# aravindr93/mjrl

Measured on AMD Instinct MI355X. Metric: NPG updates/sec (1M-timestep batch, 64x64 MLP), higher is better.
Workload: dtype f32; 1 GPU; BASELINE configs[1]: HalfCheetah-v2 shapes (obs=17, act=6), 64x64 tanh MLP, NPG 10 CG iters, 1M timesteps/batch (1000 traj x 1000), device-resident update; global_batch=1000000, parallelism=dp1 (trajectory shards, one rank sum per CG iteration: none at one rank), cg_iters=10

## Files before the change

mjrl_amd/csrc/fused_policy.h:

```cpp
#pragma once
#include <hip/hip_runtime.h>
#include <stdint.h>

#include <type_traits>
#include <vector>

namespace mjx {

typedef float f32x16 __attribute__((ext_vector_type(16)));
typedef float f32x4 __attribute__((ext_vector_type(4)));
typedef float f32x2 __attribute__((ext_vector_type(2)));

enum { MODE_VPG = 0, MODE_FVP = 1, MODE_EVAL = 2 };

struct FusedArgs {
  const float* obs;
  const float* act;
  const float* adv;
  int64_t N;
  float inv_N;
  const float* thetaA;
  const float* thetaB;
  const float* trA;
  const float* trB;
  int old_is_new;
  float* partials;
  double* spartials;
  float* dbg;
  long long* clk;
  int reverse;
  float* hcache;
  float* ocache;
  const float* snap;
  int snap_trusted;
  float* snap_out;
  int n, m;
  int raw_dr;
};

#ifdef MJX_PHASE_CLOCK
#define MJX_STAMP(k) do { __builtin_amdgcn_sched_barrier(0); if (A.dbg && blockIdx.x == 0 && wave == 0 && lane == 0 && tile == tstride) ((long long*)A.dbg)[k] = (long long)__builtin_readcyclecounter(); __builtin_amdgcn_sched_barrier(0); } while (0)
#else
#define MJX_STAMP(k) do {} while (0)
#endif
#ifdef MJX_PHASE_CLOCK
#define MJX_GSTAMP(k) do { if (A.dbg && blockIdx.x == 0 && threadIdx.x == 0) { ((long long*)A.dbg)[k] = (long long)__builtin_readcyclecounter(); ((long long*)A.dbg)[(k) + 8] = (long long)__builtin_amdgcn_s_memrealtime(); } } while (0)
#else
#define MJX_GSTAMP(k) do {} while (0)
#endif
#define MJX_MFMA(a, b, c) __builtin_amdgcn_mfma_f32_32x32x2f32((a), (b), (c), 0, 0, 0)
#define MJX_MFMA_ACC(acc, a, b) asm volatile("v_mfma_f32_32x32x2_f32 %0, %1, %2, %0" : "+a"(acc) : "v"(a), "v"(b))
#define MJX_MFMA4_ACC(acc, a, b) asm volatile("v_mfma_f32_4x4x1_16b_f32 %0, %1, %2, %0" : "+a"(acc) : "v"(a), "v"(b))
typedef __attribute__((address_space(3))) float lds_float;
__device__ __forceinline__ uint32_t lds_pin(const float* p) {
  uint32_t a = (uint32_t)(uintptr_t)(const lds_float*)p;
  asm volatile("" : "+v"(a));
  return a;
}
#define LDS_AT(addr) ((lds_float*)(uintptr_t)(addr))
#define LDS_ST(p, v) (*(p) = (v))
#define LDS_LD(p) (*(p))
#define LDS_LD2(p) (*(const f32x2*)(p))

__device__ __forceinline__ void wave_sync() {
  __builtin_amdgcn_fence(__ATOMIC_RELEASE, "wavefront");
  __builtin_amdgcn_wave_barrier();
  __builtin_amdgcn_fence(__ATOMIC_ACQUIRE, "wavefront");
}

__device__ __forceinline__ float fast_tanh(float x) {
  const float d = 1.0f + __builtin_amdgcn_exp2f(x * 2.885390081777927f);
  return fmaf(__builtin_amdgcn_rcpf(d), -2.0f, 1.0f);
}

__device__ __forceinline__ void fast_tanh16(f32x16& o, const f32x16& x) {
#pragma unroll
  for (int r = 0; r < 16; r += 2) {
    const f32x2 s = f32x2{x[r], x[r + 1]} * (f32x2)(2.885390081777927f);
    const f32x2 d = f32x2{__builtin_amdgcn_exp2f(s.x), __builtin_amdgcn_exp2f(s.y)} + (f32x2)(1.0f);
    const f32x2 rr = {__builtin_amdgcn_rcpf(d.x), __builtin_amdgcn_rcpf(d.y)};
    const f32x2 y = __builtin_elementwise_fma(rr, (f32x2)(-2.0f), (f32x2)(1.0f));
    o[r] = y.x; o[r + 1] = y.y;
  }
}

__device__ __forceinline__ float fast_div(float a, float b) {
  float r = __builtin_amdgcn_rcpf(b);
  r = r * fmaf(-b, r, 2.0f);
  return a * r;
}

__device__ __forceinline__ float half_select(uint32_t mask, float a, float b) {
  return __uint_as_float((__float_as_uint(a) & mask) | (__float_as_uint(b) & ~mask));
}

__device__ __forceinline__ float half_sum(float p) {
  auto s = __builtin_amdgcn_permlane32_swap(__float_as_uint(p), __float_as_uint(p), false, false);
  return __uint_as_float(s[0]) + __uint_as_float(s[1]);
}

__device__ __forceinline__ float row16_sum(float v) {
  auto dpp = [](float x, auto ctrl) {
    return __int_as_float(__builtin_amdgcn_update_dpp(0, __float_as_int(x), decltype(ctrl)::value, 0xF, 0xF, true));
  };
  v += dpp(v, std::integral_constant<int, 0xB1>{});
  v += dpp(v, std::integral_constant<int, 0x4E>{});
  v += dpp(v, std::integral_constant<int, 0x141>{});
  v += dpp(v, std::integral_constant<int, 0x140>{});
  return v;
}

__device__ __forceinline__ f32x16 pk_1mh2(const f32x16& h) {
  f32x16 o;
#pragma unroll
  for (int r = 0; r < 16; r += 2) {
    const f32x2 hh = {h[r], h[r + 1]};
    const f32x2 ff = __builtin_elementwise_fma(-hh, hh, (f32x2)(1.0f));
    o[r] = ff.x; o[r + 1] = ff.y;
  }
  return o;
}
__device__ __forceinline__ void pk_mul(f32x16& t, const f32x16& f) {
#pragma unroll
  for (int r = 0; r < 16; r += 2) {
    f32x2 tt = {t[r], t[r + 1]};
    tt *= f32x2{f[r], f[r + 1]};
    t[r] = tt.x; t[r + 1] = tt.y;
  }
}
__device__ __forceinline__ void pk_mul_1mh2(f32x16& t, const f32x16& h) {
#pragma unroll
  for (int r = 0; r < 16; r += 2) {
    const f32x2 hh = {h[r], h[r + 1]};
    f32x2 tt = {t[r], t[r + 1]};
    tt *= __builtin_elementwise_fma(-hh, hh, (f32x2)(1.0f));
    t[r] = tt.x; t[r + 1] = tt.y;
  }
}
__device__ __forceinline__ f32x2 pk_1mh2_pair_far(f32x2 hh) {
  f32x2 ff;
  asm("v_pk_fma_f32 %0, %1, %1, 1.0 op_sel_hi:[1,1,0] neg_lo:[1,0,0] neg_hi:[1,0,0]" : "=v"(ff) : "v"(hh));
  return ff;
}
__device__ __forceinline__ f32x16 pk_1mh2_far(const f32x16& h) {
  f32x16 o;
#pragma unroll
  for (int r = 0; r < 16; r += 2) {
    const f32x2 ff = pk_1mh2_pair_far(f32x2{h[r], h[r + 1]});
    o[r] = ff.x; o[r + 1] = ff.y;
  }
  return o;
}
__device__ __forceinline__ f32x2 mul_1mh2_pair(float a0, float a1, float h0, float h1) {
  const f32x2 ff = pk_1mh2_pair_far(f32x2{h0, h1});
  f32x2 tt = {a0, a1};
  tt *= ff;
  return tt;
}
__device__ __forceinline__ void pk_mul_1mh2_far(f32x16& t, const f32x16& h) {
#pragma unroll
  for (int r = 0; r < 16; r += 2) {
    f32x2 tt = {t[r], t[r + 1]};
    const f32x2 ff = pk_1mh2_pair_far(f32x2{h[r], h[r + 1]});
    asm("v_pk_mul_f32 %0, %0, %1" : "+v"(tt) : "v"(ff));
    t[r] = tt.x; t[r + 1] = tt.y;
  }
}

typedef __bf16 bf16x8 __attribute__((ext_vector_type(8)));
typedef uint32_t u32x4 __attribute__((ext_vector_type(4)));
#define MJX_MFMA_BF16(a, b, c) __builtin_amdgcn_mfma_f32_32x32x16_bf16(__builtin_bit_cast(bf16x8, (a)), __builtin_bit_cast(bf16x8, (b)), (c), 0, 0, 0)
struct Pc3 { u32x4 p[3]; };
__device__ __forceinline__ Pc3 split3(const float (&x)[8]) {
  Pc3 o;
#pragma unroll
  for (int k = 0; k < 4; ++k) {
    const uint32_t ua = __float_as_uint(x[2 * k]), ub = __float_as_uint(x[2 * k + 1]);
    const float ra = x[2 * k] - __uint_as_float(ua & 0xffff0000u), rb = x[2 * k + 1] - __uint_as_float(ub & 0xffff0000u);
    const uint32_t va = __float_as_uint(ra), vb = __float_as_uint(rb);
    const float la = ra - __uint_as_float(va & 0xffff0000u), lb = rb - __uint_as_float(vb & 0xffff0000u);
    o.p[0][k] = __builtin_amdgcn_perm(ub, ua, 0x07060302u);
    o.p[1][k] = __builtin_amdgcn_perm(vb, va, 0x07060302u);
    o.p[2][k] = __builtin_amdgcn_perm(__float_as_uint(lb), __float_as_uint(la), 0x07060302u);
  }
  return o;
}
__device__ __forceinline__ Pc3 split3_of(const f32x16& v, int s) {
  float x[8];
#pragma unroll
  for (int i = 0; i < 8; ++i) x[i] = v[8 * s + i];
  return split3(x);
}
__device__ __forceinline__ f32x16 mfma_bf3(const Pc3& a, const Pc3& b, f32x16 c) {
  c = MJX_MFMA_BF16(a.p[2], b.p[0], c);
  c = MJX_MFMA_BF16(a.p[0], b.p[2], c);
  c = MJX_MFMA_BF16(a.p[1], b.p[1], c);
  c = MJX_MFMA_BF16(a.p[1], b.p[0], c);
  c = MJX_MFMA_BF16(a.p[0], b.p[1], c);
  c = MJX_MFMA_BF16(a.p[0], b.p[0], c);
  return c;
}

template <int N, int I = 0, class F>
__device__ __forceinline__ void static_for(F&& f) {
  if constexpr (I < N) { f(std::integral_constant<int, I>{}); static_for<N, I + 1>(f); }
}

__device__ __forceinline__ constexpr int unit_of(int r, int hi) { return (r & 3) + 8 * (r >> 2) + 4 * hi; }

template <int H1, int H2, int NT1, int MP>
struct FusedLayout {
  static constexpr int MT1 = H1 / 32, MT2 = H2 / 32;
  static constexpr int S2 = H1 + 4;
  static constexpr int ST = 36;
  static constexpr int S3 = H2 + 4;
  static constexpr int HM = (H1 > H2 ? H1 : H2);
  int NP;
  int S1;
  int oW1, oW2, oW3, oB2, oB3, SLOT;
  int oXS, oXT, oD3, oBA, oBB, WAVE;
  int oTR, oCST, oWAVES, TOTAL;
  static constexpr int NCST = 13;
  static constexpr int F2_IMG = 3 * H1 * H2 / 2;
  __host__ __device__ explicit FusedLayout(int n, bool eval_only = false, bool bf3 = false) {
    NP = (n + 1 + 3) & ~3;
    S1 = NP + 2;
    oW1 = 0;
    oW2 = oW1 + H1 * S1;
    oW3 = oW2 + ((bf3 && H2 * S2 < F2_IMG) ? F2_IMG : H2 * S2);
    oB2 = oW3 + MP * S3;
    oB3 = oB2 + H2;
    SLOT = ((oB3 + MP + 3) / 4) * 4;
    oXS = 0;
    oXT = bf3 ? 0 : ((oXS + 32 * n + 4 * 64 + 3) / 4) * 4;
    oD3 = oXT + NP * ST;
    oBA = oD3 + MP * ST;
    oBB = oBA + HM * ST;
    WAVE = eval_only ? ((oXT + 3) / 4) * 4 : ((oBB + HM * ST + 3) / 4) * 4;
    oTR = 2 * SLOT;
    oCST = oTR + 4 * NP;
    oWAVES = oCST + NCST * MP;
    TOTAL = oWAVES + 4 * WAVE;
  }
  __host__ __device__ size_t bytes() const { return (size_t)TOTAL * 4; }
  __host__ __device__ bool fits(int n) const { return n + 1 <= 32 * NT1; }
};

struct FlatOff {
  int W1, b1, W2, b2, W3, b3, S, d;
  __host__ __device__ FlatOff(int n, int m, int h1, int h2) {
    W1 = 0; b1 = W1 + h1 * n; W2 = b1 + h1; b2 = W2 + h2 * h1; W3 = b2 + h2; b3 = W3 + m * h2; S = b3 + m; d = S + m;
  }
};

template <int H1, int H2, int NT1, int MP, int NPC>
struct RawSlab {
  static constexpr int MT1 = H1 / 32, MT2 = H2 / 32, RA = MP / 2;
  static constexpr int QPI3 = 16 / (MP / 4), UPI3 = 4 * QPI3, NT3 = H2 / UPI3;
  static constexpr int NFQ = NPC ? NPC / 4 : 1;
  static constexpr int oW2 = 0, nW2 = MT2 * MT1 * 16 * 64;
  static constexpr int oW1 = oW2 + nW2, nW1 = NPC ? MT1 * NFQ * 4 * 32 : MT1 * NT1 * 16 * 64;
  static constexpr int oW3 = oW1 + nW1, nW3 = NT3 * 4 * 64;
  static constexpr int oB2 = oW3 + nW3, nB2 = MT2 * 32;
  static constexpr int oB3 = oB2 + nB2;
  static constexpr int oS = oB3 + 2 * RA;
  static constexpr int DR = ((oS + 2 * RA) + 3) & ~3;
  static int unit(int r, int hi) { return (r & 3) + 8 * (r >> 2) + 4 * hi; }
  static bool fill_perm(int* perm, int n, int m) {
    const FlatOff fo(n, m, H1, H2);
    for (int i = 0; i < DR; ++i) perm[i] = -1;
    auto w1 = [&](int u, int f) { return f < n ? fo.W1 + u * n + f : f == n ? fo.b1 + u : -1; };
    for (int mt = 0; mt < MT2; ++mt) for (int nt = 0; nt < MT1; ++nt) for (int r = 0; r < 16; ++r) for (int l = 0; l < 64; ++l)
      perm[oW2 + ((mt * MT1 + nt) * 16 + r) * 64 + l] = fo.W2 + (32 * mt + unit(r, l >> 5)) * H1 + 32 * nt + (l & 31);
    if (NPC) {
      for (int mt = 0; mt < MT1; ++mt) for (int fq = 0; fq < NFQ; ++fq) for (int r = 0; r < 4; ++r) for (int l = 0; l < 32; ++l)
        perm[oW1 + ((mt * NFQ + fq) * 4 + r) * 32 + l] = w1(32 * mt + 4 * ((l >> 2) & 7) + r, 4 * fq + (l & 3));
    } else {
      for (int mt = 0; mt < MT1; ++mt) for (int nt = 0; nt < NT1; ++nt) for (int r = 0; r < 16; ++r) for (int l = 0; l < 64; ++l)
        perm[oW1 + ((mt * NT1 + nt) * 16 + r) * 64 + l] = w1(32 * mt + unit(r, l >> 5), 32 * nt + (l & 31));
    }
    for (int nt = 0; nt < NT3; ++nt) for (int r = 0; r < 4; ++r) for (int l = 0; l < 64; ++l) {
      const int blk = l >> 2, a = 4 * (blk / QPI3) + r, u = 4 * (blk % QPI3) + (l & 3) + UPI3 * nt;
      perm[oW3 + (nt * 4 + r) * 64 + l] = a < m ? fo.W3 + a * H2 + u : -1;
    }
    for (int nt = 0; nt < MT2; ++nt) for (int jj = 0; jj < 32; ++jj) perm[oB2 + nt * 32 + jj] = fo.b2 + 32 * nt + jj;
    for (int r = 0; r < RA; ++r) for (int hi = 0; hi < 2; ++hi) {
      const int a = unit(r, hi);
      perm[oB3 + 2 * r + hi] = a < m ? fo.b3 + a : -1;
      perm[oS + 2 * r + hi] = a < m ? fo.S + a : -1;
    }
    std::vector<int> hits(fo.d, 0);
    for (int i = 0; i < DR; ++i) if (perm[i] >= 0) { if (perm[i] >= fo.d) return false; ++hits[perm[i]]; }
    for (int i = 0; i < fo.d; ++i) if (hits[i] != 1) return false;
    return true;
  }
};

template <int H1, int H2, int NT1, int MP, int MODE, bool DBG = false, int NPC = 0, bool CACHED = false, bool BF3 = false>
__global__ __launch_bounds__(256, (MODE == MODE_EVAL && !DBG && MP <= 8) ? 2 : 1) void k_fused(FusedArgs A) {
  using LT = FusedLayout<H1, H2, NT1, MP>;
  constexpr int MT1 = LT::MT1, MT2 = LT::MT2, S2 = LT::S2, S3 = LT::S3, ST = LT::ST;
  constexpr int RA = MP / 2;
  extern __shared__ __attribute__((aligned(16))) float lds[];
  const int tid = threadIdx.x, lane = tid & 63, j = lane & 31, hi = lane >> 5;
  const int wave = __builtin_amdgcn_readfirstlane(tid >> 6);
  const uint32_t himask = hi ? 0xffffffffu : 0u;
  const int n = A.n, m = A.m;
  constexpr bool EV2 = (MODE == MODE_EVAL) && !DBG && MP <= 8;
  constexpr bool XBF3 = (MODE == MODE_FVP) && CACHED && BF3;
  static_assert(!BF3 || (CACHED && MODE == MODE_FVP && H1 == 64 && H2 == 64), "bf16x3: the cached 64 x 64 Fisher-vector product only");
  const LT L(NPC ? NPC - 1 : n, EV2, XBF3);
  const int NP = NPC ? NPC : L.NP;
  const int S1 = NP + 2;
  const FlatOff fo(n, m, H1, H2);

  float* slotA = lds;
  float* slotB = lds + L.SLOT;
  float* trs = lds + L.oTR;
  float* ws = lds + L.oWAVES + wave * L.WAVE;
  float* xs = ws + L.oXS;
  float* xT = ws + L.oXT;
  float* d3T = ws + L.oD3;
  float* bufA = ws + L.oBA;
  float* bufB = ws + L.oBB;

  MJX_GSTAMP(16);
  if (A.clk && blockIdx.x == 0 && threadIdx.x == 0) { A.clk[0] = (long long)__builtin_readcyclecounter(); A.clk[1] = (long long)__builtin_amdgcn_s_memrealtime(); }
  constexpr bool XCACHED = (MODE == MODE_FVP) && CACHED;
  constexpr int C1 = NPC ? NPC / 4 : 8 * NT1;
  constexpr int C2 = (H2 * H1 / 4 + 255) / 256;
  constexpr int C3 = (MP * H2 + 255) / 256;
  const int u1 = tid >> 2, p1 = tid & 3;
  float w1r[2][C1], w3r[2][C3], b2r[2], b3r[2], trr[4], csr[7];
  f32x4 w2r[2][C2];
#pragma unroll
  for (int s = 0; s < 2; ++s) {
    const float* th = s ? A.thetaB : A.thetaA;
    if (!(XCACHED && s == 0)) {
#pragma unroll
      for (int c = 0; c < C1; ++c) {
        const int f = p1 + 4 * c;
        const bool ok = (u1 < H1) && (f <= n);
        w1r[s][c] = th[ok ? ((f < n) ? fo.W1 + u1 * n + f : fo.b1 + u1) : 0];
      }
    }
#pragma unroll
    for (int c = 0; c < C2; ++c) { const int i4 = c * 256 + tid; w2r[s][c] = *(const f32x4*)&th[fo.W2 + 4 * (i4 < H2 * H1 / 4 ? i4 : 0)]; }
#pragma unroll
    for (int c = 0; c < C3; ++c) { const int idx = c * 256 + tid; w3r[s][c] = th[fo.W3 + (idx < m * H2 ? idx : 0)]; }
    b2r[s] = th[fo.b2 + (tid < H2 ? tid : 0)];
    b3r[s] = th[fo.b3 + (tid < m ? tid : 0)];
  }
  {
    const int i = tid < n ? tid : 0;
    trr[0] = A.trA[i]; trr[1] = A.trA[n + i]; trr[2] = A.trB[i]; trr[3] = A.trB[n + i];
    const int a = tid < m ? tid : 0;
    csr[0] = A.thetaA[fo.S + a]; csr[1] = A.thetaB[fo.S + a];
    csr[2] = A.trA[2 * n + m + a]; csr[3] = A.trA[2 * n + a];
    csr[4] = A.trB[2 * n + m + a]; csr[5] = A.trB[2 * n + a];
    csr[6] = A.thetaB[fo.b3 + a];
  }
  int mism = 0, mismx = 0;
  if (MODE == MODE_EVAL && A.ocache && !A.snap_trusted) {
    for (int idx = tid; idx < fo.d; idx += 256) mism |= (A.thetaB[idx] != A.snap[idx]);
    for (int idx = tid; idx < 2 * (n + m); idx += 256) mism |= (A.trB[idx] != A.snap[fo.d + idx]);
    if (A.hcache) for (int idx = tid; idx < 2 * n; idx += 256) mismx |= (A.trA[idx] != A.snap[fo.d + idx]);
  }
  if (MODE == MODE_VPG && A.snap_out) {
    const int nsnap = fo.d + 2 * (n + m);
    for (int idx = blockIdx.x * 256 + tid; idx < nsnap; idx += gridDim.x * 256)
      A.snap_out[idx] = idx < fo.d ? A.thetaB[idx] : A.trB[idx - fo.d];
  }
  {
    f32x4* z4 = (f32x4*)lds;
    for (int i = tid; i < L.oWAVES / 4; i += 256) z4[i] = (f32x4)(0.f);
    f32x4* w4 = (f32x4*)ws;
    for (int i = lane; i < (EV2 ? L.WAVE : L.oBA) / 4; i += 64) w4[i] = (f32x4)(0.f);
  }
  __syncthreads();
#pragma unroll
  for (int s = 0; s < 2; ++s) {
    float* slot = s ? slotB : slotA;
    if (!(XCACHED && s == 0)) {
#pragma unroll
      for (int c = 0; c < C1; ++c) {
        const int f = p1 + 4 * c;
        if ((u1 < H1) && (f <= n)) slot[L.oW1 + u1 * S1 + f] = w1r[s][c];
      }
    }
#pragma unroll
    for (int c = 0; c < C2; ++c) {
      const int i4 = c * 256 + tid;
      if (i4 < H2 * H1 / 4) *(f32x4*)&slot[L.oW2 + ((4 * i4) / H1) * S2 + (4 * i4) % H1] = w2r[s][c];
    }
#pragma unroll
    for (int c = 0; c < C3; ++c) {
      const int idx = c * 256 + tid;
      if (idx < m * H2) slot[L.oW3 + (idx / H2) * S3 + idx % H2] = w3r[s][c];
    }
    if (tid < H2) slot[L.oB2 + tid] = b2r[s];
    if (tid < m) slot[L.oB3 + tid] = b3r[s];
  }
  if (tid < n) { trs[tid] = trr[0]; trs[NP + tid] = 1.0f / (trr[1] + 1e-8f); trs[2 * NP + tid] = trr[2]; trs[3 * NP + tid] = 1.0f / (trr[3] + 1e-8f); }
  if (!EV2 && lane < 32) xT[n * ST + lane] = 1.0f;

  float* cst = lds + L.oCST;
  enum { C_OSC = 0, C_OSH = 1, C_SG = 2, C_LS = 3, C_OSCB = 4, C_OSHB = 5, C_SGB = 6, C_LSB = 7, C_DK = 8, C_ISG = 11, C_ISGB = 12,
         C_RD = 8, C_SO2 = 9, C_SN2 = 10, C_KD = 2 };
  if (tid < MP) {
    const int a = tid;
    const bool ok = a < m;
    const float lsa = ok ? csr[0] : 0.f;
    const float lsb = (ok && MODE != MODE_FVP) ? csr[1] : lsa;
    const float sga = ok ? expf(lsa) : 1.0f;
    const float dk = 2.0f / (2.0f * sga * sga + 1e-8f);
    cst[C_OSC * MP + a] = ok ? csr[2] : 0.f;
    cst[C_OSH * MP + a] = ok ? csr[3] : 0.f;
    cst[C_SG * MP + a] = sga;
    cst[C_LS * MP + a] = lsa;
    cst[C_OSCB * MP + a] = ok ? csr[4] : 0.f;
    cst[C_OSHB * MP + a] = ok ? csr[5] : 0.f;
    cst[C_SGB * MP + a] = ok ? expf(lsb) : 1.0f;
    cst[C_LSB * MP + a] = lsb;
    cst[C_DK * MP + a] = dk;
    cst[C_ISG * MP + a] = ok ? 1.0f / sga : 0.f;
    cst[C_ISGB * MP + a] = ok ? 1.0f / cst[C_SGB * MP + a] : 0.f;
    if (MODE == MODE_EVAL) {
      const float sgb = cst[C_SGB * MP + a];
      const float Dr = 2.0f * sga * sga + 1e-8f;
      float r = __builtin_amdgcn_rcpf(Dr);
      r = r * fmaf(-Dr, r, 2.0f);
      cst[C_RD * MP + a] = r;
      cst[C_SO2 * MP + a] = sgb * sgb;
      cst[C_SN2 * MP + a] = sga * sga;
      cst[C_KD * MP + a] = lsa - lsb;
    }
    if (MODE == MODE_FVP) {
      const float osc = ok ? csr[2] : 0.f;
      cst[9 * MP + 2 * a] = ok ? csr[6] : 0.f;
      cst[9 * MP + 2 * a + 1] = osc * (dk * (osc * A.inv_N));
    }
  }
  if (MODE == MODE_EVAL && mism) lds[L.oWAVES] = 1.0f;
  if (MODE == MODE_EVAL && mismx) lds[L.oWAVES + 1] = 1.0f;
  __syncthreads();
  bool use_oc = false, use_xi = false;
  if (MODE == MODE_EVAL && A.ocache) {
    use_oc = (lds[L.oWAVES] == 0.0f);
    use_xi = use_oc && NPC != 0 && A.hcache != nullptr && (lds[L.oWAVES + 1] == 0.0f);
    __syncthreads();
  }
  Pc3 w3p[XBF3 ? MT2 : 1][XBF3 ? MT1 : 1][2];
  if constexpr (XBF3) {
#pragma unroll
    for (int mt = 0; mt < MT2; ++mt)
#pragma unroll
      for (int kb = 0; kb < MT1; ++kb)
#pragma unroll
        for (int s = 0; s < 2; ++s) {
          const float* row = &slotA[L.oW2 + (32 * mt + j) * S2 + 32 * kb + 16 * s + 4 * hi];
          const f32x4 a = *(const f32x4*)row, b = *(const f32x4*)(row + 8);
          const float x[8] = {a.x, a.y, a.z, a.w, b.x, b.y, b.z, b.w};
          w3p[mt][kb][s] = split3(x);
// ... 481 lines not shown
      MJX_STAMP(6);
      f32x16 dl2s[MT2];
#pragma unroll
      for (int mt = 0; mt < MT2; ++mt) dl2s[mt] = (f32x16)(0.f);
#pragma unroll
      for (int sidx = 0; sidx < RA; ++sidx)
#pragma unroll
        for (int mt = 0; mt < MT2; ++mt) dl2s[mt] = MJX_MFMA(w6[sidx][mt], d3r[sidx], dl2s[mt]);
      float wc8[4][MT1];
      {
        const int blk = lane >> 2, g3 = blk / QPI3, uq3 = blk % QPI3;
        const float* arow = &d3T[(4 * g3 + (lane & 3)) * ST];
        const float* brow = &bufA[(4 * uq3 + (lane & 3)) * ST];
#pragma unroll
        for (int sp = 0; sp < 4; ++sp) {
          const f32x4 ave = *(const f32x4*)(arow + 8 * sp), avo = *(const f32x4*)(arow + 8 * sp + 4);
          f32x4 bve[NT3], bvo[NT3];
#pragma unroll
          for (int nt = 0; nt < NT3; ++nt) { bve[nt] = *(const f32x4*)(brow + UPI3 * nt * ST + 8 * sp); bvo[nt] = *(const f32x4*)(brow + UPI3 * nt * ST + 8 * sp + 4); }
#pragma unroll
          for (int t = 0; t < 4; ++t)
#pragma unroll
            for (int nt = 0; nt < NT3; ++nt) {
              gW3[nt] = __builtin_amdgcn_mfma_f32_4x4x1f32(ave[t], bve[nt][t], gW3[nt], 0, 0, 0);
              gW3b[nt] = __builtin_amdgcn_mfma_f32_4x4x1f32(avo[t], bvo[nt][t], gW3b[nt], 0, 0, 0);
            }
        }
        if constexpr (!XBF3) {
#pragma unroll
          for (int t = 0; t < 4; ++t)
#pragma unroll
            for (int nt = 0; nt < MT1; ++nt) wc8[t][nt] = LDS_AT(pinW[0])[t * S2 + 32 * nt];
        }
      }
      __builtin_amdgcn_sched_barrier(0);
      MJX_STAMP(7);
#pragma unroll
      for (int mt = 0; mt < MT2; ++mt) pk_mul(dl2s[mt], f2s[mt]);
      f32x16 dl1u[MT1];
      float dl2u[MT2][16];
#pragma unroll
      for (int nt = 0; nt < MT1; ++nt) dl1u[nt] = (f32x16)(0.f);
      if constexpr (XBF3) {
        __builtin_amdgcn_sched_barrier(0);
        load_h(ptile((tile + tstride < ntiles) ? tile + tstride : tile));
        const u32x4* img = (const u32x4*)(slotA + L.oW2) + lane;
        constexpr int NG8 = 2 * MT2;
        Pc3 ac = split3_of(dl2s[0], 0), an = ac, bc[MT1], bn[MT1];
#pragma unroll
        for (int nt = 0; nt < MT1; ++nt)
#pragma unroll
          for (int p = 0; p < 3; ++p) bc[nt].p[p] = img[(p * 8 + nt * 4) * 64];
        __builtin_amdgcn_sched_barrier(0);
#pragma unroll
        for (int g = 0; g < NG8; ++g) {
          if (g + 1 < NG8) {
            const int kb1 = (g + 1) >> 1, s1 = (g + 1) & 1;
#pragma unroll
            for (int nt = 0; nt < MT1; ++nt)
#pragma unroll
              for (int p = 0; p < 3; ++p) bn[nt].p[p] = img[(p * 8 + (nt * 2 + kb1) * 2 + s1) * 64];
            an = split3_of(dl2s[kb1], s1);
          }
#pragma unroll
          for (int nt = 0; nt < MT1; ++nt) dl1u[nt] = mfma_bf3(ac, bc[nt], dl1u[nt]);
          if (g < MT2) {
#pragma unroll
            for (int r = 0; r < 16; ++r) LDS_AT(pinA[4 * g + (r >> 2)])[(r & 3) * ST] = dl2s[g][r];
          } else {
            const int nt = g - MT2;
#pragma unroll
            for (int qq = 0; qq < 4; ++qq) {
              const f32x4 v = *(const f32x4*)&bufA[(32 * nt + j) * ST + 8 * qq + 4 * hi];
              dl2u[nt][4 * qq] = v.x; dl2u[nt][4 * qq + 1] = v.y; dl2u[nt][4 * qq + 2] = v.z; dl2u[nt][4 * qq + 3] = v.w;
            }
          }
          ac = an;
#pragma unroll
          for (int nt = 0; nt < MT1; ++nt) bc[nt] = bn[nt];
        }
#pragma unroll
        for (int g = 0; g < NG8; ++g)
#pragma unroll
          for (int i = 0; i < 6 * MT1; ++i) {
            __builtin_amdgcn_sched_group_barrier(0x008, 1, 0);
            if (g + 1 < NG8) {
              __builtin_amdgcn_sched_group_barrier(0x002, 4, 0);
              if (i < 3 * MT1) __builtin_amdgcn_sched_group_barrier(0x100, 1, 0);
            }
            if (g < MT2) { if (i < 4) __builtin_amdgcn_sched_group_barrier(0x200, 2, 0); else __builtin_amdgcn_sched_group_barrier(0x200, 1, 0); }
            else if (i < 4) __builtin_amdgcn_sched_group_barrier(0x100, 1, 0);
          }
        __builtin_amdgcn_sched_barrier(0);
      } else {
        constexpr int NG = MT2 * 4;
        constexpr int NGH = NG / 2;
        float wc[4][MT1], wn[4][MT1];
        __builtin_amdgcn_sched_barrier(0);
        load_h(ptile((tile + tstride < ntiles) ? tile + tstride : tile));
#pragma unroll
        for (int t = 0; t < 4; ++t)
#pragma unroll
          for (int nt = 0; nt < MT1; ++nt) wc[t][nt] = wc8[t][nt];
#pragma unroll
        for (int g = 0; g < NG; ++g) {
          const int kb = g >> 2, q = g & 3;
          if (g + 1 < NG) {
            const int kb1 = (g + 1) >> 2, q1 = (g + 1) & 3;
#pragma unroll
            for (int t = 0; t < 4; ++t)
#pragma unroll
              for (int nt = 0; nt < MT1; ++nt) wn[t][nt] = LDS_AT(pinW[4 * kb1 + q1])[t * S2 + 32 * nt];
          }
#pragma unroll
          for (int t = 0; t < 4; ++t)
#pragma unroll
            for (int nt = 0; nt < MT1; ++nt) dl1u[nt] = MJX_MFMA(dl2s[kb][4 * q + t], wc[t][nt], dl1u[nt]);
          if (g < NGH) {
            constexpr int RS = 16 * MT2 / NGH;
#pragma unroll
            for (int e = 0; e < RS; ++e) {
              const int idx = g * RS + e, mt = idx >> 4, r = idx & 15;
              LDS_AT(pinA[4 * mt + (r >> 2)])[(r & 3) * ST] = dl2s[mt][r];
            }
          } else {
            constexpr int RQ = (4 * MT2 + NGH - 1) / NGH;
#pragma unroll
            for (int e = 0; e < RQ; ++e) {
              const int idx = (g - NGH) * RQ + e;
              if (idx < 4 * MT2) {
                const int nt = idx >> 2, qq = idx & 3;
                const f32x4 v = *(const f32x4*)&bufA[(32 * nt + j) * ST + 8 * qq + 4 * hi];
                dl2u[nt][4 * qq] = v.x; dl2u[nt][4 * qq + 1] = v.y; dl2u[nt][4 * qq + 2] = v.z; dl2u[nt][4 * qq + 3] = v.w;
              }
            }
          }
#pragma unroll
          for (int t = 0; t < 4; ++t)
#pragma unroll
            for (int nt = 0; nt < MT1; ++nt) wc[t][nt] = wn[t][nt];
        }
#pragma unroll
        for (int g = 0; g < NG; ++g) {
          if (g + 1 < NG) __builtin_amdgcn_sched_group_barrier(0x100, 2 * MT1, 0);
#pragma unroll
          for (int i = 0; i < 4 * MT1; ++i) {
            __builtin_amdgcn_sched_group_barrier(0x008, 1, 0);
            if (g < NGH) __builtin_amdgcn_sched_group_barrier(0x200, 1, 0);
            else if (i < (4 * MT2 + NGH - 1) / NGH) __builtin_amdgcn_sched_group_barrier(0x100, 1, 0);
          }
        }
      }
      f32x4 bcs[4][MT1];
#pragma unroll
      for (int nt = 0; nt < MT1; ++nt) bcs[0][nt] = *(const f32x4*)&bufB[(32 * nt + j) * ST + 4 * hi];
      __builtin_amdgcn_sched_barrier(0);
      MJX_STAMP(8);
      {
#pragma unroll
        for (int q = 1; q < 4; ++q)
#pragma unroll
          for (int nt = 0; nt < MT1; ++nt) bcs[q][nt] = *(const f32x4*)&bufB[(32 * nt + j) * ST + 8 * q + 4 * hi];
#pragma unroll
        for (int q = 0; q < 4; ++q) {
#pragma unroll
          for (int t = 0; t < 4; ++t)
#pragma unroll
            for (int mt = 0; mt < MT2; ++mt)
#pragma unroll
              for (int nt = 0; nt < MT1; ++nt) MJX_MFMA_ACC(gW2[mt][nt], dl2u[mt][4 * q + t], bcs[q][nt][t]);
        }
        __builtin_amdgcn_sched_barrier(0);
      }
      MJX_STAMP(9);
#pragma unroll
      for (int nt = 0; nt < MT1; ++nt)
#pragma unroll
        for (int q = 0; q < 4; ++q)
#pragma unroll
          for (int t = 0; t < 4; t += 2) {
            const f32x2 hh = {bcs[q][nt][t], bcs[q][nt][t + 1]};
            f32x2 dd = {dl1u[nt][4 * q + t], dl1u[nt][4 * q + t + 1]};
            dd *= __builtin_elementwise_fma(-hh, hh, (f32x2)(1.0f));
            dl1u[nt][4 * q + t] = dd.x; dl1u[nt][4 * q + t + 1] = dd.y;
          }
#pragma unroll
      for (int nt = 0; nt < MT2; ++nt) {
        f32x2 s2 = {dl2u[nt][0], dl2u[nt][1]};
#pragma unroll
        for (int r = 2; r < 16; r += 2) s2 += f32x2{dl2u[nt][r], dl2u[nt][r + 1]};
        sb2[nt] += s2.x + s2.y;
      }
      __builtin_amdgcn_sched_barrier(0);
      if constexpr (NPC != 0) {
        const float* xrow = &xT[(lane & 3) * ST + 4 * hi];
#pragma unroll
        for (int q = 0; q < 4; ++q) {
          f32x4 bx[NFQ];
#pragma unroll
          for (int fq = 0; fq < NFQ; ++fq) bx[fq] = *(const f32x4*)(xrow + 4 * fq * ST + 8 * q);
#pragma unroll
          for (int t = 0; t < 4; ++t)
#pragma unroll
            for (int fq = 0; fq < NFQ; ++fq)
#pragma unroll
              for (int mt = 0; mt < MT1; ++mt)
                MJX_MFMA4_ACC(gW1q[mt][fq], dl1u[mt][4 * q + t], bx[fq][t]);
        }
      } else {
        f32x4 bc[NT1], bn[NT1];
#pragma unroll
        for (int nt = 0; nt < NT1; ++nt) { int f = 32 * nt + j; bc[nt] = *(const f32x4*)&xT[(f < NP ? f : 0) * ST + 4 * hi]; }
#pragma unroll
        for (int q = 0; q < 4; ++q) {
          if (q + 1 < 4) {
#pragma unroll
            for (int nt = 0; nt < NT1; ++nt) { int f = 32 * nt + j; bn[nt] = *(const f32x4*)&xT[(f < NP ? f : 0) * ST + 8 * (q + 1) + 4 * hi]; }
          }
#pragma unroll
          for (int nt = 0; nt < NT1; ++nt) {
            f32x4 b4 = (32 * nt + j < NP) ? bc[nt] : (f32x4)(0.f);
#pragma unroll
            for (int t = 0; t < 4; ++t)
#pragma unroll
              for (int mt = 0; mt < MT1; ++mt) gW1[mt][nt] = MJX_MFMA(dl1u[mt][4 * q + t], b4[t], gW1[mt][nt]);
          }
#pragma unroll
          for (int nt = 0; nt < NT1; ++nt) bc[nt] = bn[nt];
        }
      }
      MJX_STAMP(13);
      __builtin_amdgcn_sched_barrier(0);
    } else {
    float actr[MP], advr = 0.f;
    if (MODE != MODE_FVP) {
      if (s0 + 32 + MP <= A.N) {
        gcptr ab = ubase(A.act + s0 * m);
        gcptr db = ubase(A.adv + s0);
#pragma unroll
        for (int a = 0; a < MP; ++a) actr[a] = *(const float __attribute__((address_space(1)))*)(ab + aoff + 4 * a);
        advr = *(const float __attribute__((address_space(1)))*)(db + (uint32_t)(j * 4));
      } else {
#pragma unroll
        for (int a = 0; a < MP; ++a) actr[a] = A.act[(valid && a < m) ? (s0 + j) * m + a : 0];
        advr = A.adv[valid ? s0 + j : 0];
      }
    }
    if constexpr (DIRX) {
      const int64_t tn = tile + tstride;
      if (tn < ntiles) {
        if ((tn + 1) * 32 > A.N) set_xoff(xo, (tn * 32 + j < A.N) ? (uint32_t)j : 0u);
        load_xw(xw, xo, tn);
      }
      if (A.hcache) {
        gwptr xb = (gwptr)ubase(A.hcache + tile * HC_TILE + HC_H);
#pragma unroll
        for (int q = 0; q < NQX; ++q) *(f32x2 __attribute__((address_space(1)))*)(xb + (uint32_t)(lane * 8) + q * 512) = xn[q];
      }
    }
    if (!DIRX && !XCACHED && !XI) {
#pragma unroll
      for (int c = 0; c < XL4; ++c) {
        const int e4 = c * 64 + lane;
        *(f32x4*)&xs[4 * ((e4 < 8 * n) ? e4 : 8 * n + lane)] = xr[c];
      }
      if (tile + tstride < ntiles) load_x(tile + tstride);
      wave_sync();
    }

    auto layers12 = [&](auto tan_tag, const float* slot, const float* tsh, const float* tsc, bool writeT,
                        f32x16 (&h1)[MT1], f32x16 (&h2)[MT2], f32x16 (&t1)[MT1], f32x16 (&t2)[MT2], const f32x2 (&xdir)[NQX]) {
      constexpr bool TAN = decltype(tan_tag)::value;
      constexpr bool FWD = !(TAN && CACHED);
      f32x16 z1[MT1];
#pragma unroll
      for (int mt = 0; mt < MT1; ++mt) { z1[mt] = (f32x16)(0.f); if (TAN) t1[mt] = (f32x16)(0.f); }
      {
        f32x2 wc[MT1], vc[MT1];
        const int f00 = 2 * hi;
        auto xnorm = [&](int f) {
          const float v = (xs[j * n + f] - tsh[f]) * tsc[f];
          return (f == n) ? 1.0f : (valid ? v : 0.0f);
        };
        const float* ximg = A.hcache + tile * HC_TILE + HC_H + lane * 2;
        auto xpair = [&](int q) {
          if constexpr (TAN && CACHED) {
            if constexpr (NPC != 0) return xc[q]; else return *(const f32x2*)(ximg + q * 128);
          } else if constexpr (XI) {
            return xc[q];
          } else if constexpr (DIRX) {
            return xdir[q];
          } else {
            const int f = 4 * q + 2 * hi;
            return f32x2{xnorm(f), xnorm(f + 1)};
          }
        };
        f32x2 xb = xpair(0);
        float xb0 = xb.x, xb1 = xb.y;
#pragma unroll
        for (int mt = 0; mt < MT1; ++mt) {
          if (FWD) wc[mt] = *(const f32x2*)&slot[L.oW1 + (32 * mt + j) * S1 + f00];
          if (TAN) vc[mt] = *(const f32x2*)&slotB[L.oW1 + (32 * mt + j) * S1 + f00];
        }
#pragma unroll NPC ? NPC / 4 : 1
        for (int q = 0; q < (NPC ? NPC / 4 : NP / 4); ++q) {
          const int f0 = 4 * q + 2 * hi;
          const int f1 = (q + 1 < NP / 4) ? f0 + 4 : f0;
          f32x2 wn[MT1], vn[MT1];
          const f32x2 xnx = xpair((q + 1 < NP / 4) ? q + 1 : q);
          const float xn0 = xnx.x, xn1 = xnx.y;
          if (!DIRX && MODE == MODE_VPG && writeT && A.hcache) *(f32x2*)(A.hcache + tile * HC_TILE + HC_H + (q * 64 + lane) * 2) = f32x2{xb0, xb1};
#pragma unroll
          for (int mt = 0; mt < MT1; ++mt) {
            if (FWD) wn[mt] = *(const f32x2*)&slot[L.oW1 + (32 * mt + j) * S1 + f1];
            if (TAN) vn[mt] = *(const f32x2*)&slotB[L.oW1 + (32 * mt + j) * S1 + f1];
          }
          const float x0 = xb0, x1 = xb1;
          if (writeT) { xT[f0 * ST + j] = x0; xT[(f0 + 1) * ST + j] = x1; }
#pragma unroll
          for (int mt = 0; mt < MT1; ++mt) {
            if (FWD) z1[mt] = MJX_MFMA(wc[mt].x, x0, z1[mt]);
            if (TAN) t1[mt] = MJX_MFMA(vc[mt].x, x0, t1[mt]);
          }
#pragma unroll
          for (int mt = 0; mt < MT1; ++mt) {
            if (FWD) z1[mt] = MJX_MFMA(wc[mt].y, x1, z1[mt]);
            if (TAN) t1[mt] = MJX_MFMA(vc[mt].y, x1, t1[mt]);
          }
          xb0 = xn0; xb1 = xn1;
#pragma unroll
          for (int mt = 0; mt < MT1; ++mt) { if (FWD) wc[mt] = wn[mt]; if (TAN) vc[mt] = vn[mt]; }
        }
      }
      MJX_STAMP(2);
      if (XI && tile + tstride < ntiles) load_xi(tile + tstride);
      constexpr bool BURST = !TAN && !DBG;
      if constexpr (BURST) { __builtin_amdgcn_sched_barrier(0); if (EV2) __builtin_amdgcn_s_setprio(3); }
#pragma unroll
      for (int mt = 0; mt < MT1; ++mt) {
        if (FWD) fast_tanh16(h1[mt], z1[mt]);
        if (TAN) pk_mul_1mh2(t1[mt], h1[mt]);
      }
      if constexpr (BURST) { if (EV2) __builtin_amdgcn_s_setprio(0); __builtin_amdgcn_sched_barrier(0); }
      if (MODE == MODE_VPG && writeT && A.hcache) {
// ... 772 lines not shown
```

mjrl_amd/csrc/mjx.hip:

```cpp
#include "../../include/mjx.h"

#include <hip/hip_runtime.h>

#include <cmath>
#include <cstdarg>
#include <cstdio>
#include <cstring>
#include <pthread.h>
#include <unistd.h>
#include <atomic>
#include <string>
#include <condition_variable>
#include <functional>
#include <mutex>
#include <thread>
#include <vector>

#include "baseline.h"
#include "dynamics.h"
#include "fused_policy.h"
#include "policy_fit.h"
#include "rccl_dyn.h"
#include "launch_state.h"
#include "layerwise.h"
#include "mlp_fit.h"
#include "plan.h"
#include "vecops.h"

namespace {

thread_local std::string g_err;

int fail(int code, const char* fmt, ...) {
  char buf[512];
  va_list ap;
  va_start(ap, fmt);
  vsnprintf(buf, sizeof buf, fmt, ap);
  va_end(ap);
  g_err = buf;
  return code;
}

#define HIPCHK(expr)                                                                     \
  do {                                                                                   \
    hipError_t e_ = (expr);                                                              \
    if (e_ != hipSuccess) return fail((int)e_, "%s failed: %s (%s:%d)", #expr, hipGetErrorString(e_), __FILE__, __LINE__); \
  } while (0)

int lds_limit(const void* kern, size_t bytes) {
  const int e = mjx::dyn_lds(kern, bytes);
  if (e == mjx::LDS_OVER) return fail(MJX_ERR_UNSUPPORTED, "needs %zu + %zu static bytes of LDS (> 160 KiB)", bytes, mjx::static_lds(kern));
  if (e) return fail(e, "dynamic LDS limit of %zu bytes: %s", bytes, hipGetErrorString((hipError_t)e));
  return MJX_OK;
}
enum ScratchSite { SITE_GRAM, SITE_MLP_PREDICT, SITE_MLP_FIT, SITE_MLP_FIT_WIDE, SITE_MLP_FIT_LAUNCHES, SITE_DYN_FIT, SITE_SUM_STATS, SITE_PLAN_ROLLOUT, SITE_PLAN_SCORE };
template <class T>
int dev_scratch(ScratchSite site, void* stream, size_t bytes, T** out) {
  HIPCHK(mjx::scratch(site, (hipStream_t)stream, bytes, (void**)out));
  return MJX_OK;
}

std::atomic<long long> g_device_calls{0};
std::atomic<int> g_forked_child{0};
void atfork_child() {
  if (g_device_calls.load() > 0) g_forked_child.store(1);
  g_device_calls.store(0);
}
struct ForkGuardInit { ForkGuardInit() { pthread_atfork(nullptr, nullptr, atfork_child); } } g_fork_guard_init;

#define MJX_DEVICE_ENTRY()                                                                                                          \
  do {                                                                                                                              \
    if (g_forked_child.load())                                                                                                      \
      return fail(MJX_ERR_STATE, "libmjx: this process was forked from one that holds HIP state; device work belongs to the "      \
                                 "training process (sampler workers stay on the host, mjrl/samplers/core.py)");                     \
    g_device_calls.fetch_add(1);                                                                                                    \
  } while (0)

}

struct mjx_ctx {
  int device = 0;
  int n = 0, m = 0;
  std::vector<int> hidden;
  int64_t d = 0;
  int oS = 0;
  int n_cu = 256;
  int fused = 0;
  int grid = 256;
  size_t lds_bytes = 0;
  const float *obs = nullptr, *act = nullptr, *adv = nullptr;
  int64_t N_local = 0, N_global = 0;
  const float *theta_new = nullptr, *theta_old = nullptr, *tr_new = nullptr, *tr_old = nullptr;
  int old_is_new = 1;
  bool batch_bound = false;
  float* hcache = nullptr; size_t hcache_bytes = 0;
  bool hcache_valid = false; const float* hcache_obs = nullptr; int64_t hcache_rows = 0;
  bool ximg_ok = false; int64_t ximg_rows = 0;
  int use_hcache = 1;
  float* ocache = nullptr; size_t ocache_bytes = 0;
  float* snap = nullptr;
  bool ocache_valid = false; int64_t ocache_rows = 0;
  int64_t rows_bound = 0;
  float* partials = nullptr;
  int raw_dr = 0; int* raw_perm = nullptr;
  double* spartials = nullptr;
  float* ident_tr = nullptr;
  float *cg_x = nullptr, *cg_r = nullptr, *cg_p = nullptr, *cg_z = nullptr, *cg_Ap = nullptr;
  double* cg_scal = nullptr;
  float* dbg = nullptr;
  long long* clk = nullptr;
  unsigned fvp_seq = 0;
  bool lw_old_ok = false;
  bool prof_on = false;
  std::vector<hipEvent_t> prof_ev;
  size_t prof_used = 0;
  int prof_stride = 1;
  bool prof_iter = false;
  size_t prof_seen = 0;
  void* comm = nullptr; int comm_world = 0, comm_rank = 0;
  mjx_reduce_fn reduce_cb = nullptr; void* reduce_user = nullptr;
  struct Peer {
    bool on = false, loopback = false; int rank = 0, world = 0;
    char* buf = nullptr; char* map[16] = {nullptr};
    size_t slot_bytes = 0; uint32_t seq = 0;
    unsigned long long timeout_ticks = 500000000ull;
    int fault = 0;
  } peer;
  unsigned* ticket = nullptr;
  mjx::LayerwiseWS lw;
  mjx::LayerwiseWS lwmb;
  float *mb_x = nullptr, *mb_a = nullptr, *mb_adv = nullptr, *mb_grad = nullptr; int mb_cap = 0;
};

namespace {

using namespace mjx;

template <int H1, int H2, int NT1, int MP, bool DBG = false, int NPC = 0>
int launch_fused(mjx_ctx* c, int mode, const FusedArgs& a, hipStream_t st) {
  const bool ev2 = (mode == MODE_EVAL) && MP <= 8;
  const bool cached = (mode == MODE_FVP) && a.hcache != nullptr && !DBG;
  static const bool bf3_on = env_flag("MJX_FVP_BF16X3", true);
  constexpr bool BF3_OK = H1 == 64 && H2 == 64 && MP == 8;
  const bool bf3 = BF3_OK && cached && bf3_on && FusedLayout<H1, H2, NT1, MP>(NPC ? NPC - 1 : c->n, false, true).bytes() <= LDS_MAX;
  FusedLayout<H1, H2, NT1, MP> L(NPC ? NPC - 1 : c->n, ev2, bf3);
  size_t bytes = L.bytes();
  void (*k)(FusedArgs) = nullptr;
  if (mode == MODE_VPG) k = k_fused<H1, H2, NT1, MP, MODE_VPG, DBG, NPC>;
  else if (mode == MODE_FVP) k = cached ? k_fused<H1, H2, NT1, MP, MODE_FVP, false, NPC, true> : k_fused<H1, H2, NT1, MP, MODE_FVP, DBG, NPC>;
  else k = k_fused<H1, H2, NT1, MP, MODE_EVAL, false, NPC>;
  if constexpr (BF3_OK) { if (bf3) k = k_fused<H1, H2, NT1, MP, MODE_FVP, false, NPC, true, true>; }
  if (cached) mode = 3;
  if (int rc = lds_limit((const void*)k, bytes)) return rc;
  hipLaunchKernelGGL(k, dim3(ev2 ? 2 * c->grid : c->grid), dim3(256), bytes, st, a);
  HIPCHK(hipGetLastError());
  return MJX_OK;
}

int npc_of(int fused, int n) {
  const int NPr = (n + 1 + 3) & ~3;
#ifdef MJX_PHASE_CLOCK
  return (fused == 1 && NPr == 20) ? 20 : 0;
#else
  return (fused == 1 && (NPr == 20 || NPr == 12 || NPr == 8)) ? NPr : 0;
#endif
}
int raw_slab(int fused, int npc, int n, int m, std::vector<int>* perm) {
  auto one = [&](auto rs) -> int {
    using RS = decltype(rs);
    if (perm) { perm->assign(RS::DR, -1); if (!RS::fill_perm(perm->data(), n, m)) return 0; }
    return RS::DR;
  };
  switch (fused) {
    case 1: return npc == 20 ? one(RawSlab<64, 64, 1, 8, 20>{}) : npc == 12 ? one(RawSlab<64, 64, 1, 8, 12>{}) : npc == 8 ? one(RawSlab<64, 64, 1, 8, 8>{})
                                                                                                                             : one(RawSlab<64, 64, 1, 8, 0>{});
    case 2: return one(RawSlab<32, 32, 1, 8, 0>{});
    case 3: return one(RawSlab<64, 64, 1, 16, 0>{});
    case 4: return one(RawSlab<32, 32, 1, 16, 0>{});
    case 5: return one(RawSlab<32, 32, 2, 8, 0>{});
    case 6: return one(RawSlab<32, 32, 2, 32, 0>{});
  }
  return 0;
}

template <int H1, int H2, int NT1, int MP>
bool variant_fits(int n, int m, int h1, int h2, int64_t d, size_t* bytes) {
  if (h1 != H1 || h2 != H2 || m > MP || n + 1 > 32 * NT1) return false;
  FusedLayout<H1, H2, NT1, MP> L(n);
  if (L.bytes() > LDS_MAX) return false;
  if ((size_t)(4 * d + 64) * 4 > L.bytes()) return false;
  *bytes = L.bytes();
  return true;
}

int pick_variant(int n, int m, const std::vector<int>& hid, int64_t d, size_t* bytes) {
  if (hid.size() != 2) return 0;
  int h1 = hid[0], h2 = hid[1];
  if (variant_fits<64, 64, 1, 8>(n, m, h1, h2, d, bytes)) return 1;
  if (variant_fits<32, 32, 1, 8>(n, m, h1, h2, d, bytes)) return 2;
  if (variant_fits<64, 64, 1, 16>(n, m, h1, h2, d, bytes)) return 3;
  if (variant_fits<32, 32, 1, 16>(n, m, h1, h2, d, bytes)) return 4;
  if (variant_fits<32, 32, 2, 8>(n, m, h1, h2, d, bytes)) return 5;
  if (variant_fits<32, 32, 2, 32>(n, m, h1, h2, d, bytes)) return 6;
  return 0;
}

int dispatch_fused(mjx_ctx* c, int mode, const FusedArgs& a, hipStream_t st) {
  const int NPr = (c->n + 1 + 3) & ~3;
#ifdef MJX_PHASE_CLOCK
  if (c->fused == 1 && NPr == 20) return launch_fused<64, 64, 1, 8, false, 20>(c, mode, a, st);
#endif
  if (c->fused == 1 && NPr == 20 && !c->dbg) return launch_fused<64, 64, 1, 8, false, 20>(c, mode, a, st);
  if (c->fused == 1 && NPr == 12 && !c->dbg) return launch_fused<64, 64, 1, 8, false, 12>(c, mode, a, st);
  if (c->fused == 1 && NPr == 8 && !c->dbg) return launch_fused<64, 64, 1, 8, false, 8>(c, mode, a, st);
  switch (c->fused) {
#ifdef MJX_PHASE_CLOCK
    case 1: return launch_fused<64, 64, 1, 8>(c, mode, a, st);
#else
    case 1: return c->dbg ? launch_fused<64, 64, 1, 8, true>(c, mode, a, st) : launch_fused<64, 64, 1, 8>(c, mode, a, st);
#endif
    case 2: return launch_fused<32, 32, 1, 8>(c, mode, a, st);
    case 3: return launch_fused<64, 64, 1, 16>(c, mode, a, st);
    case 4: return launch_fused<32, 32, 1, 16>(c, mode, a, st);
    case 5: return launch_fused<32, 32, 2, 8>(c, mode, a, st);
    case 6: return launch_fused<32, 32, 2, 32>(c, mode, a, st);
  }
  return fail(MJX_ERR_STATE, "no fused variant");
}

FusedArgs make_args(mjx_ctx* c, const float* thetaB) {
  FusedArgs a;
  a.obs = c->obs; a.act = c->act; a.adv = c->adv;
  a.N = c->N_local;
  a.inv_N = (float)(1.0 / (double)c->N_global);
  a.thetaA = c->theta_new; a.thetaB = thetaB;
  a.trA = c->tr_new ? c->tr_new : c->ident_tr;
  a.trB = c->tr_old ? c->tr_old : c->ident_tr;
  a.old_is_new = c->old_is_new;
  a.partials = c->partials; a.spartials = c->spartials;
  a.dbg = c->dbg;
  a.clk = c->clk;
  a.reverse = 0;
  a.hcache = nullptr; a.ocache = nullptr; a.snap = nullptr; a.snap_out = nullptr; a.snap_trusted = 0;
  a.n = c->n; a.m = c->m;
#ifdef MJX_PHASE_CLOCK
  a.raw_dr = c->raw_perm ? c->raw_dr : 0;
#else
  a.raw_dr = (c->raw_perm && !c->dbg) ? c->raw_dr : 0;
#endif
  return a;
}

int check_bound(mjx_ctx* c, bool need_act) {
  if (!c) return fail(MJX_ERR_ARG, "null context");
  if (!c->batch_bound || c->N_local < 0 || c->N_global <= 0) return fail(MJX_ERR_STATE, "mjx_bind_batch has not been called");
  if (need_act && c->N_local > 0 && (!c->act || !c->adv)) return fail(MJX_ERR_STATE, "actions / advantages not bound");
  if (!c->theta_new || !c->theta_old) return fail(MJX_ERR_STATE, "mjx_bind_policy has not been called");
  return MJX_OK;
}

}

extern "C" {

const char* mjx_last_error(void) { return g_err.c_str(); }
int mjx_version(void) { return 1; }

int mjx_process_state(int64_t* out2) {
  if (!out2) return fail(MJX_ERR_ARG, "null output");
  out2[0] = (int64_t)g_device_calls.load();
  out2[1] = (int64_t)g_forked_child.load();
  return MJX_OK;
}

int mjx_device_count(void) {
  if (g_forked_child.load()) return 0;
  g_device_calls.fetch_add(1);
  int n = 0;
  if (hipGetDeviceCount(&n) != hipSuccess) { (void)hipGetLastError(); return 0; }
  return n;
}

int mjx_create(mjx_ctx** out, int device, int n, int m, const int* hidden, int n_hidden) {
  if (!out || n <= 0 || m <= 0 || n_hidden < 0 || (n_hidden > 0 && !hidden)) return fail(MJX_ERR_ARG, "bad arguments");
  MJX_DEVICE_ENTRY();
  if (mjx_device_count() <= device) return fail(MJX_ERR_NOGPU, "HIP device %d not available", device);
  HIPCHK(hipSetDevice(device));
  mjx_ctx* c = new mjx_ctx();
  c->device = device; c->n = n; c->m = m;
  c->hidden.assign(hidden, hidden + n_hidden);
  int prev = n; int64_t d = 0;
  for (int h : c->hidden) { if (h <= 0) { delete c; return fail(MJX_ERR_ARG, "bad hidden size"); } d += (int64_t)prev * h + h; prev = h; }
  d += (int64_t)prev * m + m;
  c->oS = (int)d;
  d += m;
  c->d = d;
  c->n_cu = cu_count();
  c->grid = c->n_cu;
  c->fused = pick_variant(n, m, c->hidden, d, &c->lds_bytes);
  if (env_flag("MJX_FORCE_LAYERWISE", false)) c->fused = 0;
  if (env_flag("MJX_NO_HCACHE", false)) c->use_hcache = 0;
  if (c->fused) {
    std::vector<int> perm;
    const int dr = !env_flag("MJX_RAW_SLAB", true) ? 0 : raw_slab(c->fused, npc_of(c->fused, n), n, m, &perm);
// ... 1307 lines not shown
```

Before: 309.8 updates/s.

## Interleave bf16x3 splitting and bias sums with W2-gradient MFMAs in cached FVP

Adds a new bf16x3 variant of the cached Fisher-vector-product kernel, on by default through an env flag. It computes the W2 gradient with explicit accumulator-register bf16 MFMAs. The bf16 splitting of the second K-half and the layer-1 activation reloads are software-pipelined between those MFMAs, and the b2 bias reduction is moved ahead of the MFMA loop. The aim is to hide the VALU split work and LDS loads under matrix-core latency. The cost is higher register pressure from holding current and next split operands, plus inserted s_nop hazards in inline asm.

```diff
diff --git a/mjrl_amd/csrc/fused_policy.h b/mjrl_amd/csrc/fused_policy.h
--- a/mjrl_amd/csrc/fused_policy.h
+++ b/mjrl_amd/csrc/fused_policy.h
@@ -51,6 +51,7 @@
 #define MJX_MFMA(a, b, c) __builtin_amdgcn_mfma_f32_32x32x2f32((a), (b), (c), 0, 0, 0)
 #define MJX_MFMA_ACC(acc, a, b) asm volatile("v_mfma_f32_32x32x2_f32 %0, %1, %2, %0" : "+a"(acc) : "v"(a), "v"(b))
 #define MJX_MFMA4_ACC(acc, a, b) asm volatile("v_mfma_f32_4x4x1_16b_f32 %0, %1, %2, %0" : "+a"(acc) : "v"(a), "v"(b))
+#define MJX_MFMA_BF16_ACC(acc, a, b) asm volatile("s_nop 1\n\tv_mfma_f32_32x32x16_bf16 %0, %1, %2, %0" : "+a"(acc) : "v"(a), "v"(b))
 typedef __attribute__((address_space(3))) float lds_float;
 __device__ __forceinline__ uint32_t lds_pin(const float* p) {
   uint32_t a = (uint32_t)(uintptr_t)(const lds_float*)p;
@@ -171,18 +172,19 @@
 typedef uint32_t u32x4 __attribute__((ext_vector_type(4)));
 #define MJX_MFMA_BF16(a, b, c) __builtin_amdgcn_mfma_f32_32x32x16_bf16(__builtin_bit_cast(bf16x8, (a)), __builtin_bit_cast(bf16x8, (b)), (c), 0, 0, 0)
 struct Pc3 { u32x4 p[3]; };
+__device__ __forceinline__ void split3_pair(Pc3& o, int k, float xa, float xb) {
+  const uint32_t ua = __float_as_uint(xa), ub = __float_as_uint(xb);
+  const float ra = xa - __uint_as_float(ua & 0xffff0000u), rb = xb - __uint_as_float(ub & 0xffff0000u);
+  const uint32_t va = __float_as_uint(ra), vb = __float_as_uint(rb);
+  const float la = ra - __uint_as_float(va & 0xffff0000u), lb = rb - __uint_as_float(vb & 0xffff0000u);
+  o.p[0][k] = __builtin_amdgcn_perm(ub, ua, 0x07060302u);
+  o.p[1][k] = __builtin_amdgcn_perm(vb, va, 0x07060302u);
+  o.p[2][k] = __builtin_amdgcn_perm(__float_as_uint(lb), __float_as_uint(la), 0x07060302u);
+}
 __device__ __forceinline__ Pc3 split3(const float (&x)[8]) {
   Pc3 o;
 #pragma unroll
-  for (int k = 0; k < 4; ++k) {
-    const uint32_t ua = __float_as_uint(x[2 * k]), ub = __float_as_uint(x[2 * k + 1]);
-    const float ra = x[2 * k] - __uint_as_float(ua & 0xffff0000u), rb = x[2 * k + 1] - __uint_as_float(ub & 0xffff0000u);
-    const uint32_t va = __float_as_uint(ra), vb = __float_as_uint(rb);
-    const float la = ra - __uint_as_float(va & 0xffff0000u), lb = rb - __uint_as_float(vb & 0xffff0000u);
-    o.p[0][k] = __builtin_amdgcn_perm(ub, ua, 0x07060302u);
-    o.p[1][k] = __builtin_amdgcn_perm(vb, va, 0x07060302u);
-    o.p[2][k] = __builtin_amdgcn_perm(__float_as_uint(lb), __float_as_uint(la), 0x07060302u);
-  }
+  for (int k = 0; k < 4; ++k) split3_pair(o, k, x[2 * k], x[2 * k + 1]);
   return o;
 }
 __device__ __forceinline__ Pc3 split3_of(const f32x16& v, int s) {
@@ -296,7 +298,7 @@
   }
 };
 
-template <int H1, int H2, int NT1, int MP, int MODE, bool DBG = false, int NPC = 0, bool CACHED = false, bool BF3 = false>
+template <int H1, int H2, int NT1, int MP, int MODE, bool DBG = false, int NPC = 0, bool CACHED = false, bool BF3 = false, bool BF3R9 = false>
 __global__ __launch_bounds__(256, (MODE == MODE_EVAL && !DBG && MP <= 8) ? 2 : 1) void k_fused(FusedArgs A) {
   using LT = FusedLayout<H1, H2, NT1, MP>;
   constexpr int MT1 = LT::MT1, MT2 = LT::MT2, S2 = LT::S2, S3 = LT::S3, ST = LT::ST;
@@ -309,6 +311,8 @@
   constexpr bool EV2 = (MODE == MODE_EVAL) && !DBG && MP <= 8;
   constexpr bool XBF3 = (MODE == MODE_FVP) && CACHED && BF3;
   static_assert(!BF3 || (CACHED && MODE == MODE_FVP && H1 == 64 && H2 == 64), "bf16x3: the cached 64 x 64 Fisher-vector product only");
+  constexpr bool XR9 = XBF3 && BF3R9;
+  static_assert(!BF3R9 || BF3, "bf16x3 R9: an option of the bf16x3 kernel");
   const LT L(NPC ? NPC - 1 : n, EV2, XBF3);
   const int NP = NPC ? NPC : L.NP;
   const int S1 = NP + 2;
@@ -1096,11 +1100,73 @@
         }
       }
       f32x4 bcs[4][MT1];
-#pragma unroll
-      for (int nt = 0; nt < MT1; ++nt) bcs[0][nt] = *(const f32x4*)&bufB[(32 * nt + j) * ST + 4 * hi];
-      __builtin_amdgcn_sched_barrier(0);
-      MJX_STAMP(8);
-      {
+      if constexpr (XR9) {
+        f32x4 hq[4][MT1];
+#pragma unroll
+        for (int q = 0; q < 2; ++q)
+#pragma unroll
+          for (int nt = 0; nt < MT1; ++nt) hq[q][nt] = *(const f32x4*)&bufB[(32 * nt + j) * ST + 8 * q + 4 * hi];
+        __builtin_amdgcn_sched_barrier(0);
+        MJX_STAMP(8);
+#pragma unroll
+        for (int nt = 0; nt < MT2; ++nt) {
+          f32x2 s2 = {dl2u[nt][0], dl2u[nt][1]};
+#pragma unroll
+          for (int r = 2; r < 16; r += 2) s2 += f32x2{dl2u[nt][r], dl2u[nt][r + 1]};
+          sb2[nt] += s2.x + s2.y;
+        }
+        Pc3 ac[MT2], bc[MT1], an[MT2], bn[MT1];
+#pragma unroll
+        for (int mt = 0; mt < MT2; ++mt)
+#pragma unroll
+          for (int k = 0; k < 4; ++k) split3_pair(ac[mt], k, dl2u[mt][2 * k], dl2u[mt][2 * k + 1]);
+#pragma unroll
+        for (int nt = 0; nt < MT1; ++nt)
+#pragma unroll
+          for (int k = 0; k < 4; ++k) split3_pair(bc[nt], k, hq[k >> 1][nt][(2 * k) & 3], hq[k >> 1][nt][(2 * k + 1) & 3]);
+        __builtin_amdgcn_sched_barrier(0);
+#pragma unroll
+        for (int s = 0; s < 2; ++s) {
+          if (s == 0) {
+#pragma unroll
+            for (int q = 2; q < 4; ++q)
+#pragma unroll
+              for (int nt = 0; nt < MT1; ++nt) hq[q][nt] = *(const f32x4*)&bufB[(32 * nt + j) * ST + 8 * q + 4 * hi];
+          }
+#pragma unroll
+          for (int p = 0; p < 6; ++p) {
+            const int pa = p == 0 ? 2 : (p == 2 || p == 3) ? 1 : 0, pb = p == 1 ? 2 : (p == 2 || p == 4) ? 1 : 0;
+#pragma unroll
+            for (int mt = 0; mt < MT2; ++mt)
+#pragma unroll
+              for (int nt = 0; nt < MT1; ++nt) {
+                MJX_MFMA_BF16_ACC(gW2[mt][nt], ac[mt].p[pa], bc[nt].p[pb]);
+                const int i = (p * MT2 + mt) * MT1 + nt;
+                if (s == 0) {
+                  if (i < 4 * (MT2 + MT1)) {
+                    const int o = i >> 2, k = i & 3;
+                    if (o < MT2) split3_pair(an[o], k, dl2u[o][8 + 2 * k], dl2u[o][8 + 2 * k + 1]);
+                    else split3_pair(bn[o - MT2], k, hq[2 + (k >> 1)][o - MT2][(2 * k) & 3], hq[2 + (k >> 1)][o - MT2][(2 * k + 1) & 3]);
+                  }
+                } else if (i < 4 * MT1) {
+                  const int q = i / MT1, n2 = i % MT1;
+                  bcs[q][n2] = *(const f32x4*)&bufB[(32 * n2 + j) * ST + 8 * q + 4 * hi];
+                }
+                __builtin_amdgcn_sched_barrier(0);
+              }
+          }
+          if (s == 0) {
+#pragma unroll
+            for (int mt = 0; mt < MT2; ++mt) ac[mt] = an[mt];
+#pragma unroll
+            for (int nt = 0; nt < MT1; ++nt) bc[nt] = bn[nt];
+          }
+        }
+      } else {
+#pragma unroll
+        for (int nt = 0; nt < MT1; ++nt) bcs[0][nt] = *(const f32x4*)&bufB[(32 * nt + j) * ST + 4 * hi];
+        __builtin_amdgcn_sched_barrier(0);
+        MJX_STAMP(8);
 #pragma unroll
         for (int q = 1; q < 4; ++q)
 #pragma unroll
@@ -1128,12 +1194,14 @@
             dd *= __builtin_elementwise_fma(-hh, hh, (f32x2)(1.0f));
             dl1u[nt][4 * q + t] = dd.x; dl1u[nt][4 * q + t + 1] = dd.y;
           }
-#pragma unroll
-      for (int nt = 0; nt < MT2; ++nt) {
-        f32x2 s2 = {dl2u[nt][0], dl2u[nt][1]};
-#pragma unroll
-        for (int r = 2; r < 16; r += 2) s2 += f32x2{dl2u[nt][r], dl2u[nt][r + 1]};
-        sb2[nt] += s2.x + s2.y;
+      if constexpr (!XR9) {
+#pragma unroll
+        for (int nt = 0; nt < MT2; ++nt) {
+          f32x2 s2 = {dl2u[nt][0], dl2u[nt][1]};
+#pragma unroll
+          for (int r = 2; r < 16; r += 2) s2 += f32x2{dl2u[nt][r], dl2u[nt][r + 1]};
+          sb2[nt] += s2.x + s2.y;
+        }
       }
       __builtin_amdgcn_sched_barrier(0);
       if constexpr (NPC != 0) {
diff --git a/mjrl_amd/csrc/mjx.hip b/mjrl_amd/csrc/mjx.hip
--- a/mjrl_amd/csrc/mjx.hip
+++ b/mjrl_amd/csrc/mjx.hip
@@ -149,7 +149,10 @@
   if (mode == MODE_VPG) k = k_fused<H1, H2, NT1, MP, MODE_VPG, DBG, NPC>;
   else if (mode == MODE_FVP) k = cached ? k_fused<H1, H2, NT1, MP, MODE_FVP, false, NPC, true> : k_fused<H1, H2, NT1, MP, MODE_FVP, DBG, NPC>;
   else k = k_fused<H1, H2, NT1, MP, MODE_EVAL, false, NPC>;
-  if constexpr (BF3_OK) { if (bf3) k = k_fused<H1, H2, NT1, MP, MODE_FVP, false, NPC, true, true>; }
+  static const bool bf3_r9_on = env_flag("MJX_FVP_BF16X3_R9", true);
+  if constexpr (BF3_OK) {
+    if (bf3) k = bf3_r9_on ? k_fused<H1, H2, NT1, MP, MODE_FVP, false, NPC, true, true, true> : k_fused<H1, H2, NT1, MP, MODE_FVP, false, NPC, true, true>;
+  }
   if (cached) mode = 3;
   if (int rc = lds_limit((const void*)k, bytes)) return rc;
   hipLaunchKernelGGL(k, dim3(ev2 ? 2 * c->grid : c->grid), dim3(256), bytes, st, a);
```

New measurement: 317.7 updates/s (median of 6 runs). +2.5%, better.
